# automl/mdp-playground

Measured on AMD Instinct MI355X. Metric: env-steps/sec, higher is better.
Workload: dtype u8; 1 GPU; cfg2: BASELINE configs[1]: discrete 8x8, delay 4, sequence_length 3; 65536 envs/GPU, random actions, same-step autoreset; 1 bench step = 1 fused launch of 512 env steps; envs_per_gpu=65536, fuse=512, env_steps_per_bench_step=33554432, rng=numpy, collective=all_gather_into_tensor(nccl, 1 rank) after every launch

## Files before the change

mdp_playground_amd/csrc/mdpp_discrete_lean.hip:

```cpp
#include <stdlib.h>

#include <stdio.h>

#include <type_traits>

#ifndef MDPP_LEAN_TU_NEXT
#define MDPP_LEAN_TU_NEXT 0
#endif
#ifndef MDPP_LEAN_TU_NOISE
#define MDPP_LEAN_TU_NOISE 0
#endif

#include "mdpp_internal.hpp"
#include "mdpp_rng.hpp"

namespace mdpp {

#ifndef MDPP_LEAN_CHUNK
#define MDPP_LEAN_CHUNK 8
#endif
#ifndef MDPP_LEAN_DEPTH
#define MDPP_LEAN_DEPTH 32
#endif
#ifndef MDPP_LEAN_AHEAD
#define MDPP_LEAN_AHEAD 4
#endif
#if defined(MDPP_LEAN_PRIO_E) || defined(MDPP_LEAN_PRIO_O) || defined(MDPP_LEAN_PRIO_H)
#define MDPP_LEAN_PRIO_FORCED 1
#else
#define MDPP_LEAN_PRIO_FORCED 0
#endif
#ifndef MDPP_LEAN_PRIO_E
#define MDPP_LEAN_PRIO_E 3
#endif
#ifndef MDPP_LEAN_PRIO_O
#define MDPP_LEAN_PRIO_O 2
#endif
#ifndef MDPP_LEAN_PRIO_H
#define MDPP_LEAN_PRIO_H 0
#endif
#ifndef MDPP_LEAN_PRIO_O2
#define MDPP_LEAN_PRIO_O2 -1
#endif
#ifndef MDPP_LEAN_ST_AUX
#define MDPP_LEAN_ST_AUX MDPP_ST_NT
#endif
#ifndef MDPP_LEAN_ST_AUX_BYTES
#define MDPP_LEAN_ST_AUX_BYTES MDPP_LEAN_ST_AUX
#endif
#ifndef MDPP_LEAN_LD_AUX
#define MDPP_LEAN_LD_AUX 0
#endif
#ifndef MDPP_LEAN_HMIN
#define MDPP_LEAN_HMIN 16
#endif
#ifndef MDPP_LEAN_HSLEEP
#define MDPP_LEAN_HSLEEP 8
#endif
namespace lean {
constexpr int kChunk = MDPP_LEAN_CHUNK;
constexpr int kDepth = MDPP_LEAN_DEPTH;
constexpr int kAhead = MDPP_LEAN_AHEAD;
constexpr int kPRsrc = 0x00020000;
constexpr uint32_t kSpinLimit = 1u << 22;
constexpr uint32_t kStatusInternal = 0x80000000u;
constexpr uint32_t kQueueCap = 6;
constexpr int kHChunks = 8;
constexpr int kHChunksNp = 4;
constexpr int kXR = 16;
constexpr int kXB = 4;
constexpr int kDepthNp = 16;
constexpr int kRoles = 4;
constexpr uint32_t kSelPad = 0x0c0c0c00u;
typedef unsigned int u32x2 __attribute__((ext_vector_type(2)));
typedef unsigned int u32x4 __attribute__((ext_vector_type(4)));

__device__ __forceinline__ uint32_t wg_load_acq(const uint32_t *p) {
    return __hip_atomic_load(p, __ATOMIC_ACQUIRE, __HIP_MEMORY_SCOPE_WORKGROUP);
}
__device__ __forceinline__ void wg_store_rel(uint32_t *p, uint32_t v) {
    __hip_atomic_store(p, v, __ATOMIC_RELEASE, __HIP_MEMORY_SCOPE_WORKGROUP);
}
__device__ __forceinline__ void chunk_words(uint64_t seed, uint64_t genv, uint64_t b0, uint32_t r4, uint32_t stream,
                                            uint32_t (&wd)[MDPP_LEAN_CHUNK]) {
    uint32_t o0[4], o1[4], o2[4] = {0u, 0u, 0u, 0u};
    philox_start_block(seed, genv, b0, stream, o0);
    philox_start_block(seed, genv, b0 + 1, stream, o1);
    if (r4 != 0u) philox_start_block(seed, genv, b0 + 2, stream, o2);
    const uint32_t all[12] = {o0[0], o0[1], o0[2], o0[3], o1[0], o1[1], o1[2], o1[3], o2[0], o2[1], o2[2], o2[3]};
#pragma unroll
// ... 4 lines not shown
                                              float (&z)[MDPP_LEAN_CHUNK]) {
    float all[12] = {0.0f, 0.0f, 0.0f, 0.0f, 0.0f, 0.0f, 0.0f, 0.0f, 0.0f, 0.0f, 0.0f, 0.0f};
    uint32_t o[4];
    philox_start_block(seed, genv, b0, stream, o);
    philox_box_muller2(o, all[0], all[1], all[2], all[3]);
    philox_start_block(seed, genv, b0 + 1, stream, o);
    philox_box_muller2(o, all[4], all[5], all[6], all[7]);
    if (r4 != 0u) {
        philox_start_block(seed, genv, b0 + 2, stream, o);
        philox_box_muller2(o, all[8], all[9], all[10], all[11]);
    }
#pragma unroll
    for (int u = 0; u < MDPP_LEAN_CHUNK; u++)
        z[u] = r4 == 0u ? all[u] : r4 == 1u ? all[u + 1] : r4 == 2u ? all[u + 2] : all[u + 3];
}
}
using namespace lean;

template <bool OBS64, bool DELAY, bool HASMAX, bool EVN, bool PHILOX, bool IRR, bool NEXT, int NZ = 0>
__global__ __launch_bounds__(kRoles * kBlock) void k_discrete_rollout_lean(DiscreteArgs a, int K,
                                                                      const int32_t *__restrict__ actions,
                                                                      void *__restrict__ obs,
                                                                      float *__restrict__ reward,
                                                                      uint8_t *__restrict__ term,
                                                                      uint8_t *__restrict__ trunc,
                                                                      void *__restrict__ final_obs) {
    const uint64_t ptick0 = tick_now(a);
    constexpr bool PN = (NZ & 1) != 0, RN = (NZ & 2) != 0;
    constexpr bool NPN = PN && !PHILOX, NRN = RN && !PHILOX;
    constexpr bool Z0 = (NZ & 4) != 0;
    static_assert(!Z0 || NRN, "sigma-0 draws: numpy streams with the reward_noise key");
    constexpr bool NRX = NRN && !Z0;
    constexpr int KD = NRN ? kDepthNp : kDepth;
    __shared__ __align__(16) uint32_t lds_rec[3][KD][kBlock];
    __shared__ __align__(16) uint32_t lds_V[2048];
    __shared__ __align__(16) uint2 lds_col[16];
    __shared__ __align__(16) uint32_t lds_R[128];
    __shared__ __align__(16) uint64_t lds_T[8];
    __shared__ __align__(16) float lds_rsel[EVN ? 4 * 64 : 4];
    __shared__ __align__(16) uint64_t lds_ring[kBlock];
    __shared__ uint32_t lds_head[kBlock];
    __shared__ uint32_t lds_prod[kBlock / 64];
    __shared__ __align__(8) uint32_t lds_cons[kBlock / 64][2];
    __shared__ uint32_t lds_done;
    constexpr bool ROWS2 = !IRR && NZ == 0;
    constexpr bool ROWS1 = ROWS2 && !PHILOX;
    constexpr int kRB = 4;
    __shared__ __align__(16) float lds_rw[ROWS1 ? kRB : 1][kChunk][ROWS1 ? kBlock : 4];
    __shared__ __align__(16) uint32_t lds_rprod[kBlock / 64], lds_rcons[kBlock / 64];
    typedef typename std::conditional<IRR, uint64_t, uint32_t>::type S0Word;
    __shared__ __align__(16) S0Word lds_s0[PHILOX ? kHChunks : 1][kBlock];
    __shared__ __align__(16) uint2 lds_col1[IRR ? 16 : 1];
    __shared__ __align__(16) uint64_t lds_T1[IRR ? 8 : 1];
    __shared__ uint32_t lds_hprod[kBlock / 64];
    __shared__ uint32_t lds_pprod[kBlock / 64];
    constexpr bool kNpNoise = !PHILOX && NZ != 0;
    constexpr bool kPhNoise = PHILOX && NZ != 0;
    constexpr int kPrioE = MDPP_LEAN_PRIO_FORCED ? MDPP_LEAN_PRIO_E : kNpNoise ? 2 : !PHILOX ? MDPP_LEAN_PRIO_E : 1;
    constexpr int kPrioO = MDPP_LEAN_PRIO_FORCED ? MDPP_LEAN_PRIO_O : kNpNoise ? 1 : !PHILOX ? MDPP_LEAN_PRIO_O : kPhNoise ? 2 : (PN ? 2 : 3);
    constexpr int kPrioH = MDPP_LEAN_PRIO_FORCED ? MDPP_LEAN_PRIO_H : kNpNoise ? 3 : !PHILOX ? MDPP_LEAN_PRIO_H : kPhNoise ? 2 : (PN ? 3 : 2);
    static_assert(NZ == 0 || (!IRR && !NEXT), "noise on the lean kernel: one sub-space, same-step autoreset");
    __shared__ __align__(16) uint32_t lds_pn[(PN && PHILOX) ? kHChunks : 1][kBlock];
    __shared__ __align__(16) uint32_t lds_pn2[NPN ? kHChunksNp : 1][2][kBlock];
    __shared__ __align__(16) double lds_x[NRX ? kXR : 1][kBlock];
    __shared__ uint16_t lds_meta[NRN ? kXR : 1][kBlock];
    __shared__ __align__(16) double lds_rx[NRX ? KD : 1][kBlock];
    __shared__ uint32_t lds_hhead[NRN ? kBlock : 1], lds_epos[NRN ? kBlock : 1];
    __shared__ uint8_t lds_sstab[(NRN || NPN) ? 2048 : 1];
    __shared__ uint8_t lds_pntab[NPN ? 4096 : 1];
    __shared__ ulonglong2 lds_kw[NRN ? 256 : 1];
    __shared__ double lds_fi[NRN ? 256 : 1];
    constexpr int kEN = IRR ? 2 : 1;
    constexpr bool nextmode = NEXT;
    const bool ar = a.autoreset != 0;
    const int tid = threadIdx.x;
    const int role = tid / kBlock;
    const int l = tid & (kBlock - 1);
    const int w = l >> 6;
    const uint32_t S = (uint32_t)a.S, L = (uint32_t)a.L;
    if (tid < 16) {
        uint64_t cs = 0;
        if (tid < a.A)
            for (uint32_t s = 0; s < S; s++) {
                const uint32_t nx = a.P[s * a.A + tid] & 7u;
                cs |= (uint64_t)(nx | 8u | ((uint32_t)((a.term_mask >> nx) & 1ULL) << 7)) << (8 * s);
            }
        lds_col[tid] = make_uint2((uint32_t)cs, (uint32_t)(cs >> 32));
        if (tid < 8) lds_T[tid] = a.init_thr[tid];
        if (IRR) {
            uint64_t c1 = 0;
            if (tid < a.A1)
                for (int s1 = 0; s1 < a.S1; s1++) c1 |= (uint64_t)(a.P1[s1 * a.A1 + tid] & 7u) << (8 * s1);
            lds_col1[tid] = make_uint2((uint32_t)c1, (uint32_t)(c1 >> 32));
            if (tid < 8) lds_T1[tid] = tid < a.S1 ? (uint64_t)ceil(a.init_cdf1[tid] * 9007199254740992.0) : ~0ULL;
        }
        if (!EVN && tid < 4) lds_rsel[tid] = a.rsel[tid];
    }
    if (EVN)
        for (int k = tid; k < 4 * a.every_n; k += kRoles * kBlock) lds_rsel[k] = a.rsel[k < 4 ? k : (k & 1)];
    for (uint32_t k = tid; k < 128; k += kRoles * kBlock) {
        uint32_t wd = 0;
        for (int b = 0; b < 4; b++) {
            uint32_t byte = 4 * k + b;
            if (byte < a.rbits_stride) wd |= (uint32_t)a.rbits[byte] << (8 * b);
        }
        lds_R[k] = wd;
    }
    if (tid < kBlock) { lds_ring[tid] = 0; lds_head[tid] = 0; if (NRN) { lds_hhead[tid] = 0; lds_epos[tid] = 0; } }
    if (NRN || NPN) {
        for (uint32_t k = tid; k < 2048u; k += kRoles * kBlock) {
            const uint64_t lo = (uint64_t)k << 53, hi = lo + ((1ULL << 53) - 1ULL);
            uint32_t c0 = 0, c1 = 0;
            for (int j = 0; j < 8; j++) {
                const uint64_t t = a.init_thr[j] > (1ULL << 53) - 1ULL ? ~0ULL : a.init_thr[j] << 11;
                c0 += (t <= lo) ? 1u : 0u; c1 += (t <= hi) ? 1u : 0u;
            }
            lds_sstab[k] = (uint8_t)(c0 == c1 ? c0 : 0xFFu);
        }
    }
    if (NPN) {
        for (uint32_t k = tid; k < 4096u; k += kRoles * kBlock) {
            const uint64_t lo = (uint64_t)k << 52, hi = lo + ((1ULL << 52) - 1ULL);
            uint32_t a0 = 0, a1 = 0, b0 = 0, b1 = 0;
            for (int j = 0; j < 7; j++) { a0 += (a.pn_TL[j] <= lo) ? 1u : 0u; a1 += (a.pn_TL[j] <= hi) ? 1u : 0u; }
            for (int j = 0; j < 8; j++) { b0 += (a.pn_TU[j] <= lo) ? 1u : 0u; b1 += (a.pn_TU[j] <= hi) ? 1u : 0u; }
            lds_pntab[k] = (uint8_t)((a0 == a1 && b0 == b1) ? (a0 | (b0 << 4)) : 0xFFu);
        }
    }
    if (NRN)
        for (int k = tid; k < 256; k += kRoles * kBlock) { lds_kw[k] = make_ulonglong2(d_zig_ki[k], (unsigned long long)(__double_as_longlong(d_zig_wi[k]) + (52LL << 52)));    lds_fi[k] = d_zig_fi[k]; }
    if (tid < kBlock / 64) { lds_prod[tid] = 0; lds_cons[tid][0] = 0; lds_cons[tid][1] = 0; lds_hprod[tid] = 0; lds_pprod[tid] = 0; lds_rprod[tid] = 0; lds_rcons[tid] = 0; }
    if (tid == 0) lds_done = 0;
    __syncthreads();
    {
        uint32_t dmask = 0;
        for (uint32_t j = 1; j <= L; j++) dmask |= 1u << (4 * j - 2);
        for (uint32_t d = tid; d < 2048; d += kRoles * kBlock) {
            uint32_t wd = 0;
            if ((d & dmask) == dmask) {
                for (uint32_t b = 8; b < 32; b++) {
                    if (!(b & 8u)) continue;
                    const uint32_t idx = d * 32u + b;
// ... 5 lines not shown
            lds_V[d] = wd;
        }
    }
    uint32_t steps_at_launch = 0;
    {
        const uint32_t eb0 = ((gridDim.x & 7u) == 0u) ? (blockIdx.x & 7u) * (gridDim.x >> 3) + (blockIdx.x >> 3) : blockIdx.x;
        const uint32_t i0 = eb0 * kBlock + l;
        if (EVN && role == 1 && i0 < (uint32_t)a.N) steps_at_launch = ((const uint32_t *)&a.state[i0])[2] & 0x7FFFFFFFu;
    }
    __syncthreads();

    const uint32_t eblk = ((gridDim.x & 7u) == 0u) ? (blockIdx.x & 7u) * (gridDim.x >> 3) + (blockIdx.x >> 3) : blockIdx.x;
    const uint32_t i = eblk * kBlock + l;
    const uint32_t N = (uint32_t)a.N;
    const bool rows = ROWS2 && (N % (uint32_t)kBlock) == 0u;
    const uint32_t blk0 = eblk * kBlock, ln = (uint32_t)l & 63u;
    const uint32_t ws = (uint32_t)__builtin_amdgcn_readfirstlane(w);
    auto min4 = [&](const uint32_t *p) -> uint32_t {
        const uint64_t x = __hip_atomic_load((const uint64_t *)p, __ATOMIC_ACQUIRE, __HIP_MEMORY_SCOPE_WORKGROUP);
        const uint64_t y = __hip_atomic_load((const uint64_t *)p + 1, __ATOMIC_ACQUIRE, __HIP_MEMORY_SCOPE_WORKGROUP);
        return min(min((uint32_t)x, (uint32_t)(x >> 32)), min((uint32_t)y, (uint32_t)(y >> 32)));
    };
    if (i >= N) {
        if (role == 0 && (l & 63) == 0) __hip_atomic_fetch_add(&lds_done, 1u, __ATOMIC_RELEASE, __HIP_MEMORY_SCOPE_WORKGROUP);
        return;
    }
    const uint32_t A = (uint32_t)a.A;
    constexpr int kMinLanes = MDPP_LEAN_HMIN;
    uint32_t status = 0;

    if (role == 3) {
        if (!ar && !PN && !NRN) return;
        __builtin_amdgcn_s_setprio(kPrioH);
        if constexpr (PHILOX) {
            const uint64_t genv = (uint64_t)(a.env_id_offset + (int64_t)i);
            const int nch = (K + kChunk - 1) / kChunk;
            static_assert(kChunk == 8, "two start-state blocks per chunk");
            uint32_t thr[8], thr1[8];
#pragma unroll
            for (int j = 0; j < 8; j++) {
                const uint64_t t53 = lds_T[j];
                thr[j] = __builtin_amdgcn_readfirstlane(t53 > (1ULL << 53) ? 0x80000000u : (uint32_t)((t53 + 0x3FFFFFULL) >> 22));
                const uint64_t u53 = IRR ? lds_T1[j] : ~0ULL;
                thr1[j] = __builtin_amdgcn_readfirstlane(u53 > (1ULL << 53) ? 0x80000000u : (uint32_t)((u53 + 0x3FFFFFULL) >> 22));
            }
            const uint32_t r4 = (uint32_t)ptick0 & 3u;
            for (int c = 0; c < nch; c++) {
                if (c >= kHChunks) {
                    const uint32_t must = (uint32_t)min((c - kHChunks + 1) * kChunk, K);
                    uint32_t spins = 0;
                    while (wg_load_acq(&lds_prod[w]) < must) {
                        __builtin_amdgcn_s_sleep(2);
                        if (++spins > kSpinLimit) { status |= kStatusInternal; break; }
                    }
                }
                const uint64_t b0 = (ptick0 + (uint64_t)(c * kChunk)) >> 2;
                auto words = [&](uint32_t stream, uint32_t (&wd)[kChunk]) { chunk_words(a.philox_seed, genv, b0, r4, stream, wd); };
                uint32_t wd[kChunk], wd1[kChunk];
                words(kPhiloxStartStream, wd);
                if (IRR) words(kPhiloxStartIrrStream, wd1);
                S0Word pk = 0;
#pragma unroll
                for (int u = 0; u < kChunk; u++) {
                    const uint32_t m = wd[u] >> 1;
                    uint32_t s0 = 0;
#pragma unroll
                    for (int j = 0; j < 7; j++) s0 += (thr[j] <= m) ? 1u : 0u;
                    if (IRR) {
                        const uint32_t m1 = wd1[u] >> 1;
                        uint32_t s1 = 0;
#pragma unroll
                        for (int j = 0; j < 7; j++) s1 += (thr1[j] <= m1) ? 1u : 0u;
                        s0 |= (s1 | 8u) << 4;
                    }
                    pk |= (S0Word)(s0 | 8u) << (kEN * 4 * u);
                }
                lds_s0[c % kHChunks][l] = pk;
                if ((l & 63) == 0) wg_store_rel(&lds_hprod[w], (uint32_t)(c + 1));
            }
            if (status) atomicOr(&a.status[i], status);
            return;
        }
        if constexpr (NPN || NRN) {
            Pcg64 g;
            g.load(a.env_s, a.env_inc, i);
            Pcg64LimbsLo ge;
            ge.from(g);
            uint32_t hq = 0;
            uint64_t look = 0;
            if (NRN) look = ge.next64();
            uint32_t vals = 0, tail = 0, spins = 0;
            auto start_of = [&](uint64_t r) __attribute__((always_inline)) -> uint32_t {
                uint32_t s0 = lds_sstab[(uint32_t)(r >> 53)];
                if (__builtin_expect(__builtin_amdgcn_ballot_w64(s0 == 0xFFu) != 0, 0)) {
                    if (s0 == 0xFFu) {
                        const uint64_t m = r >> 11;
                        s0 = 0;
#pragma unroll
                        for (int j = 0; j < 8; j++) s0 += (a.init_thr[j] <= m) ? 1u : 0u;
                    }
                }
                return s0;
            };
            for (;;) {
                if (wg_load_acq(&lds_done) == kBlock / 64) break;
                bool did = false;
                if constexpr (NRN) {
                    const uint32_t epos = __hip_atomic_load(&lds_epos[l], __ATOMIC_RELAXED, __HIP_MEMORY_SCOPE_WORKGROUP);
                    const bool go = hq + (uint32_t)kXB <= epos + (uint32_t)kXR;
                    if (__builtin_amdgcn_ballot_w64(go) != 0) {
                        uint32_t rej = 0;
                        uint64_t wdv[kXB + 1];
                        if (go) {
                            wdv[0] = look;
#pragma unroll
                            for (int u = 0; u < kXB; u++) {
                                const uint64_t wd = wdv[u];
                                wdv[u + 1] = ge.next64();
                                const uint64_t rabs = (wd >> 9) & 0x000fffffffffffffULL;
                                if constexpr (Z0) {
                                    const uint64_t ki = lds_kw[(uint32_t)wd & 0xffu].x;
                                    const bool ok = rabs < ki;
                                    rej |= ok ? 0u : (1u << u);
                                    lds_meta[(hq + (uint32_t)u) & (uint32_t)(kXR - 1)][l] = (uint16_t)(start_of(wd) | (ok ? 0u : (2u << 3)));
                                    continue;
                                }
                                const ulonglong2 kw = lds_kw[(uint32_t)wd & 0xffu];
                                const double W = __longlong_as_double((long long)kw.y);
                                const double x = __builtin_fma(__longlong_as_double((long long)(rabs | 0x3FF0000000000000ULL)), W, -W);
                                const uint64_t xb = (uint64_t)__double_as_longlong(x);
                                const double xs = __longlong_as_double((long long)(((uint64_t)(((uint32_t)(xb >> 32) & 0x7FFFFFFFu) |
                                                                                   (((uint32_t)wd << 23) & 0x80000000u)) << 32) | (uint32_t)xb));
                                const bool ok = rabs < kw.x;
                                rej |= ok ? 0u : (1u << u);
                                const uint32_t slot = (hq + (uint32_t)u) & (uint32_t)(kXR - 1);
                                lds_x[slot][l] = xs;
// ... 77 lines not shown
                            tail += 1u;
                        }
                        __hip_atomic_store(&lds_ring[l], (uint64_t)vals | ((uint64_t)tail << 32), __ATOMIC_RELEASE,
                                           __HIP_MEMORY_SCOPE_WORKGROUP);
                        did = true;
                    }
                }
                if (__builtin_amdgcn_ballot_w64(did) == 0) {
                    __builtin_amdgcn_s_sleep(2);
                    if (++spins > kSpinLimit * 4u) { status |= kStatusInternal; break; }
                } else {
                    spins = 0;
                }
            }
            auto undraw = [&](Pcg64 &gg, uint32_t q) {
                for (; q > 0; q--) {
                    uint64_t lo = gg.s_lo - gg.inc_lo;
                    uint64_t hi = gg.s_hi - gg.inc_hi - (gg.s_lo < gg.inc_lo ? 1ULL : 0ULL);
                    gg.s_lo = lo * a.minv_lo;
                    gg.s_hi = __umul64hi(lo, a.minv_lo) + lo * a.minv_hi + hi * a.minv_lo;
                }
            };
            ge.to(g);
            if (NRN) undraw(g, hq + 1u - __hip_atomic_load(&lds_epos[l], __ATOMIC_ACQUIRE, __HIP_MEMORY_SCOPE_WORKGROUP));
            else undraw(g, tail - wg_load_acq(&lds_head[l]));
            g.store(a.env_s, i);
            if (status) atomicOr(&a.status[i], status);
            return;
        }
        Pcg64 g;
        g.load(a.env_s, a.env_inc, i);
        auto draw = [&](Pcg64 &gg) -> uint32_t {
            const uint64_t r0 = gg.next64();
            const uint64_t m = r0 >> 11;
            uint32_t s0 = 0;
#pragma unroll
            for (int j = 0; j < 8; j++) s0 += (lds_T[j] <= m) ? 1u : 0u;
            if (IRR) {
                const uint64_t m1 = gg.next64() >> 11;
                uint32_t s1 = 0;
#pragma unroll
                for (int j = 0; j < 8; j++) s1 += (lds_T1[j] <= m1) ? 1u : 0u;
                s0 |= (s1 | 8u) << 4;
            }
            return s0;
        };
        uint32_t vals = 0, tail = 0;
        for (;;) {
            if (wg_load_acq(&lds_done) == kBlock / 64) break;
            const uint32_t head = wg_load_acq(&lds_head[l]);
            const uint32_t cnt = tail - head;
            const bool want = cnt + (uint32_t)kEN <= 8u;
            const uint64_t bw = __builtin_amdgcn_ballot_w64(want);
            const bool urgent = __builtin_amdgcn_ballot_w64(want && cnt <= 2) != 0;
            if (__builtin_popcountll(bw) >= kMinLanes || urgent) {
                Pcg64 n = g;
                const uint32_t s0 = draw(n) | 8u;
                if (want) {
                    const uint32_t sh = (tail & 7u) * 4u;
                    g = n;
                    vals = (vals & ~((IRR ? 0xFFu : 0xFu) << sh)) | (s0 << sh);
                    tail += (uint32_t)kEN;
                }
                __hip_atomic_store(&lds_ring[l], (uint64_t)vals | ((uint64_t)tail << 32), __ATOMIC_RELEASE,
                                   __HIP_MEMORY_SCOPE_WORKGROUP);
            } else {
                __builtin_amdgcn_s_sleep(MDPP_LEAN_HSLEEP);
            }
        }
        const uint32_t head = wg_load_acq(&lds_head[l]);
        for (uint32_t q = tail - head; q > 0; q--) {
            uint64_t lo = g.s_lo - g.inc_lo;
            uint64_t hi = g.s_hi - g.inc_hi - (g.s_lo < g.inc_lo ? 1ULL : 0ULL);
            g.s_lo = lo * a.minv_lo;
            g.s_hi = __umul64hi(lo, a.minv_lo) + lo * a.minv_hi + hi * a.minv_lo;
        }
        g.store(a.env_s, i);
        return;
    }

    const uint32_t total = (uint32_t)K * N;
    const int nchunks = (K + kChunk - 1) / kChunk;

    if (role == 1) {
        __builtin_amdgcn_s_setprio(kPrioO);
        auto r_rew = __builtin_amdgcn_make_buffer_rsrc((void *)reward, 0, total * 4u, kPRsrc);
        const uint32_t v4 = i * 4u;
        const uint32_t dsh = (uint32_t)(a.delay > 0 ? a.delay - 1 : 0);
        uint32_t ring = ((const uint32_t *)&a.state[i])[3];
        const uint8_t *rselb = (const uint8_t *)lds_rsel;

        const uint32_t ph_full = 16u * (uint32_t)a.every_n;
        uint32_t ph = EVN ? ph_full - 16u * (steps_at_launch % (uint32_t)a.every_n) : 0u;
        const uint64_t genv = (uint64_t)(a.env_id_offset + (int64_t)i);
        const uint32_t r4 = (uint32_t)ptick0 & 3u;
        float zc[kChunk] = {0.0f, 0.0f, 0.0f, 0.0f, 0.0f, 0.0f, 0.0f, 0.0f};
        const bool plain = a.scale == 1.0 && a.shift == 0.0;
        auto emit = [&](uint32_t ra, uint32_t rb, uint32_t rc, uint32_t so, double z, float *stage) {
            uint32_t bit = lds_V[(ra >> 5) & 2047u] >> (ra & 31u);
            uint32_t out;
            if (DELAY) {
                out = (ring >> dsh) & 1u;
                ring = (ring << 1) | (bit & 1u);
                ring = (ra != rb) ? 0u : ring;
            } else {
                out = bit & 1u;
            }
            const uint32_t tb = (rc >> 7) & 1u;
            uint32_t rd = 0;
            if (EVN) {
                ph -= 16u;
                rd = ph;
                ph = (ra != rb || ph == 0u) ? ph_full : ph;
            }
            float rout;
            if constexpr (RN && !Z0) {
                double r = (out != 0u && (!EVN || rd == 0u)) ? 1.0 : 0.0;
                r += 0.0 + a.r_noise * z;
                if (!plain) {
                    r *= a.scale;
                    r += a.shift;
                }
                if (tb) r += a.term_add;
                rout = (float)r;
            } else {
                rout = EVN ? *(const float *)(rselb + (rd | (out << 3) | (tb << 2)))
                           : *(const float *)(rselb + (((out << 1) | tb) << 2));
            }
            if (nextmode) rout = (ra != rb) ? 0.0f : rout;
            if (stage) { *stage = rout; return; }
            __builtin_amdgcn_raw_buffer_store_b32(__float_as_uint(rout), r_rew, v4, so * 4u, MDPP_LEAN_ST_AUX);
        };
        for (int c = 0; c < nchunks; c++) {
            const int kbase = c * kChunk;
            const uint32_t upto = (uint32_t)min(kbase + kChunk, K);
            if constexpr (RN && PHILOX)
                chunk_normals(a.philox_seed, genv, (ptick0 + (uint64_t)kbase) >> 2, r4, kPhiloxRNoiseStream, zc);
            uint32_t spins = 0;
            while (wg_load_acq(&lds_prod[w]) < upto) {
                __builtin_amdgcn_s_sleep(1);
                if (++spins > kSpinLimit) { status |= kStatusInternal; break; }
            }
            const bool rowc = ROWS1 && rows && kbase + kChunk <= K;
            if (kbase + kChunk <= K) {
                uint32_t ra[kChunk], rb[kChunk], rc[kChunk];
#pragma unroll
                for (int u = 0; u < kChunk; u++) {
                    ra[u] = lds_rec[0][(kbase + u) % KD][l];
                    rb[u] = lds_rec[1][(kbase + u) % KD][l];
                    rc[u] = lds_rec[2][(kbase + u) % KD][l];
                }
                double zd[kChunk];
#pragma unroll
                for (int u = 0; u < kChunk; u++) zd[u] = NRX ? lds_rx[NRX ? (kbase + u) % KD : 0][l] : (double)zc[u];
                if (rowc && c >= kRB) {
                    uint32_t sp2 = 0;
                    while (min4(lds_rcons) < (uint32_t)(c - kRB + 1)) {
                        __builtin_amdgcn_s_sleep(1);
                        if (++sp2 > kSpinLimit) { status |= kStatusInternal; break; }
                    }
                }
#pragma unroll
                for (int u = 0; u < kChunk; u++)
                    emit(ra[u], rb[u], rc[u], (uint32_t)(kbase + u) * N, zd[u], rowc ? &lds_rw[ROWS1 ? (c % kRB) : 0][u][ROWS1 ? l : 0] : nullptr);
            } else {
#pragma unroll
                for (int u = 0; u < kChunk; u++)
                    if (kbase + u < K)
                        emit(lds_rec[0][(kbase + u) % KD][l], lds_rec[1][(kbase + u) % KD][l],
                             lds_rec[2][(kbase + u) % KD][l], (uint32_t)(kbase + u) * N,
                             NRX ? lds_rx[NRX ? (kbase + u) % KD : 0][l] : (double)zc[u], nullptr);
            }
            if ((l & 63) == 0) wg_store_rel(&lds_cons[w][0], upto);
            if constexpr (ROWS1) {
                if (rowc && (l & 63) == 0) wg_store_rel(&lds_rprod[w], (uint32_t)(c + 1));
            }
        }
        ((uint32_t *)&a.state[i])[3] = ring;
        if (status) atomicOr(&a.status[i], status);
        return;
    }

    if (role == 2) {
        __builtin_amdgcn_s_setprio(MDPP_LEAN_PRIO_O2 >= 0 ? MDPP_LEAN_PRIO_O2 : (NPN && !MDPP_LEAN_PRIO_FORCED) ? (NRN ? 2 : 3)
                                   : (PN && PHILOX && !MDPP_LEAN_PRIO_FORCED) ? (RN ? 2 : 3) : kPrioO);
        auto r_obs = __builtin_amdgcn_make_buffer_rsrc(obs, 0, total * (OBS64 ? 8u : 4u) * (uint32_t)kEN, kPRsrc);
        auto r_term = __builtin_amdgcn_make_buffer_rsrc((void *)term, 0, total, kPRsrc);
        auto r_rew2 = __builtin_amdgcn_make_buffer_rsrc((void *)reward, 0, total * 4u, kPRsrc);
        auto r_trunc = __builtin_amdgcn_make_buffer_rsrc((void *)trunc, 0, total, kPRsrc);
        const uint32_t v1 = i, v4 = i * 4u, v8 = i * 8u, v16 = i * 16u;
        auto emit = [&](uint32_t rb, uint32_t rc, uint32_t so) {
            const uint32_t o = rb & 7u;
            if (IRR) {
                const uint32_t o1 = (rc >> 8) & 7u;
                if (OBS64) __builtin_amdgcn_raw_buffer_store_b128(u32x4{o, 0u, o1, 0u}, r_obs, v16 + so * 16u, 0, MDPP_LEAN_ST_AUX);
                else __builtin_amdgcn_raw_buffer_store_b64(u32x2{o, o1}, r_obs, v8, so * 8u, MDPP_LEAN_ST_AUX);
            } else if (OBS64) __builtin_amdgcn_raw_buffer_store_b64(u32x2{o, 0u}, r_obs, v8, so * 8u, MDPP_LEAN_ST_AUX);
            else __builtin_amdgcn_raw_buffer_store_b32(o, r_obs, v4, so * 4u, MDPP_LEAN_ST_AUX);
            __builtin_amdgcn_raw_buffer_store_b8((uint8_t)((rc >> 7) & 1u), r_term, v1, so, MDPP_LEAN_ST_AUX_BYTES);
            __builtin_amdgcn_raw_buffer_store_b8(HASMAX ? (uint8_t)(rc >> 16) : (uint8_t)0, r_trunc, v1, so, MDPP_LEAN_ST_AUX_BYTES);
        };
        Pcg64 sp;
// ... 188 lines not shown
        }
        if constexpr (NRN) return;
        if (!PHILOX && !ar) return;
        if constexpr (PHILOX) {
            uint32_t spins = 0;
            while (wg_load_acq(&lds_hprod[w]) < (uint32_t)(c + 1)) {
                __builtin_amdgcn_s_sleep(1);
                if (++spins > kSpinLimit) { status |= kStatusInternal; break; }
            }
            s0c = lds_s0[c % kHChunks][l];
            if constexpr (PN) {
                spins = 0;
                while (wg_load_acq(&lds_pprod[w]) < (uint32_t)(c + 1)) {
                    __builtin_amdgcn_s_sleep(1);
                    if (++spins > kSpinLimit) { status |= kStatusInternal; break; }
                }
                pnc = lds_pn[c % kHChunks][l];
            }
            return;
        }
        const uint64_t rt = __hip_atomic_load(&lds_ring[l], __ATOMIC_ACQUIRE, __HIP_MEMORY_SCOPE_WORKGROUP);
        const uint32_t vals = (uint32_t)rt, tail = (uint32_t)(rt >> 32);
        const uint32_t qc = (uint32_t)__builtin_popcount(qv & 0x88888888u);
        const uint32_t avail = tail - head_local, room = kQueueCap - qc;
        const uint32_t take = avail < room ? avail : room;
        const uint32_t rot = __builtin_amdgcn_alignbit(vals, vals, (head_local & 7u) * 4u);
        const uint32_t m = (1u << (4u * take)) - 1u;
        qv |= (rot & m) << (4u * qc);
        head_local += take;
        __hip_atomic_store(&lds_head[l], head_local, __ATOMIC_RELAXED, __HIP_MEMORY_SCOPE_WORKGROUP);
    };
    typedef typename std::conditional<IRR, uint2, int>::type Act;
    typedef typename std::conditional<IRR, uint4, uint2>::type Col;
    auto column = [&](Act act, uint32_t &badm, int u) -> Col {
        int action;
        if constexpr (IRR) action = (int)act.x; else action = act;
        uint32_t ua = (uint32_t)action;
        if (__builtin_expect(__builtin_amdgcn_ballot_w64(ua >= A) != 0, 0)) {
            ua = (uint32_t)(action + ((action >> 31) & (int)A));
            const bool bad = ua >= A;
            if (nextmode) badm |= bad ? (1u << u) : 0u; else status |= bad ? (uint32_t)MDPP_STATUS_BAD_ACTION : 0u;
            ua = bad ? 0u : ua;
        }
        if constexpr (IRR) {
            const int action1 = (int)act.y;
            uint32_t ub = (uint32_t)action1;
            if (__builtin_expect(__builtin_amdgcn_ballot_w64(ub >= A1) != 0, 0)) {
                ub = (uint32_t)(action1 + ((action1 >> 31) & (int)A1));
                const bool bad = ub >= A1;
                if (nextmode) badm |= bad ? (1u << u) : 0u; else status |= bad ? (uint32_t)MDPP_STATUS_BAD_ACTION : 0u;
                ub = bad ? 0u : ub;
            }
            const uint2 ca = lds_col[ua], cb = lds_col1[ub];
            return make_uint4(ca.x, ca.y, cb.x, cb.y);
        } else {
            return lds_col[ua];
        }
    };
    auto stepE = [&](const Col &col, int k, uint32_t badbit) {
        uint32_t entry = __builtin_amdgcn_perm(col.y, col.x, sel);
        if constexpr (PN && PHILOX) {
            const uint32_t nib = (pnc >> (4 * (k % kChunk))) & 0xFu, j = nib & 7u, nx = entry & 7u;
            const uint32_t ns = nib > 7u ? j + (j >= nx ? 1u : 0u) : nx;
            entry = __builtin_amdgcn_perm(enc_hi, enc_lo, ns | kSelPad);
        }
        if constexpr (NPN) {
            const uint32_t by = (((k % kChunk) < 4 ? pnc : pnc_hi) >> (8 * (k & 3))) & 0xFFu, nx = entry & 7u;
            const uint32_t ns = min(by & 15u, nx) + (uint32_t)max((int)(by >> 4) - (int)nx, 0);
            entry = __builtin_amdgcn_perm(enc_hi, enc_lo, ns | kSelPad);
        }
        const uint32_t k2n = (k2 << 4) | entry;
        bool need = entry > 0x7Fu;
        uint32_t rc = entry;
        if (HASMAX) {
            cnt += 1;
            need = need || cnt >= 0x10000u;
            rc = __builtin_amdgcn_perm(cnt, entry, 0x0c060c00u);
        }
        need = need && ar;
        uint32_t rec_a = k2n;
        if (nextmode) {
            const bool ended = need && !pend;
            need = pend;
            rc = pend ? 0u : rc;
            rec_a = pend ? 0u : k2n;
            status |= (badbit != 0u && !pend) ? (uint32_t)MDPP_STATUS_BAD_ACTION : 0u;
            pend = ended;
        }
        uint32_t s0v = PHILOX ? (uint32_t)(s0c >> (kEN * 4 * (k % kChunk))) & (IRR ? 0xFFu : 0xFu) : qv & (IRR ? 0xFFu : 0xFu);
        if constexpr (NRN) {
            uint32_t kind = (m0 >> 3) & 3u;
            if (__builtin_expect(__builtin_amdgcn_ballot_w64(kind >= 2u) != 0, 0)) {
                uint32_t guard = 0;
                while (__builtin_amdgcn_ballot_w64(kind == 2u) != 0) {
                    const bool red = kind == 2u;
                    ep += red ? 2u : 0u;
                    uint32_t o0 = m0, o1 = m1, o2 = m2;
                    double ox = xv;
                    fetch();
                    if (!red) { m0 = o0; m1 = o1; m2 = o2; xv = ox; }
                    kind = (m0 >> 3) & 3u;
                    if (++guard > 64u) { status |= kStatusInternal; break; }
                }
            }
            uint32_t cntw = kind == 0u ? 1u : 2u, ssm = kind == 0u ? m1 : m2;
            if (kind == 3u) { cntw = m0 >> 8; ssm = m0 >> 5; }
            if constexpr (NRX) lds_rx[k % KD][l] = xv;
            s0v = (ssm & 7u) | 8u;
            ep += cntw + (need ? 1u : 0u);
            __hip_atomic_store(&lds_epos[l], ep, __ATOMIC_RELAXED, __HIP_MEMORY_SCOPE_WORKGROUP);
            fetch();
        }
        if (!PHILOX && !NRN && __builtin_expect(__builtin_amdgcn_ballot_w64(need && s0v == 0u) != 0, 0)) {
            uint32_t spins = 0;
            while (__builtin_amdgcn_ballot_w64(need && (qv & 0xFu) == 0u) != 0) {
                pull(-1);
                __builtin_amdgcn_s_sleep(1);
                if (++spins > kSpinLimit) { status |= kStatusInternal; qv |= 8u; break; }
            }
            s0v = qv & (IRR ? 0xFFu : 0xFu);
        }
        if constexpr (IRR) {
            const uint32_t n1 = __builtin_amdgcn_perm(col.w, col.z, c1 | kSelPad);
            c1 = need ? ((s0v >> 4) & 7u) : n1;
            rc |= c1 << 8;
            s0v &= 0xFu;
        }
        k2 = need ? s0v : k2n;
        if (!PHILOX && !NRN) qv = need ? (qv >> (4 * kEN)) : qv;
        if (HASMAX) cnt = need ? c0 : cnt;
        else last_reset = need ? (uint32_t)(k + 1) : last_reset;
        sel = (k2 & 7u) | kSelPad;
        lds_rec[0][k % KD][l] = rec_a;
        lds_rec[1][k % KD][l] = k2;
        lds_rec[2][k % KD][l] = rc;
    };

    auto load_act = [&](int k) -> Act {
        const uint32_t kk = (uint32_t)min(k, K - 1);
        if constexpr (IRR) {
            const u32x2 v = __builtin_amdgcn_raw_buffer_load_b64(r_act, v4, kk * N * 8u, MDPP_LEAN_LD_AUX);
            return make_uint2(v.x, v.y);
        } else {
            return __builtin_amdgcn_raw_buffer_load_b32(r_act, v4, kk * N * 4u, MDPP_LEAN_LD_AUX);
        }
    };
    constexpr int kAh = IRR ? 2 : kAhead;
    static_assert(kAh % 2 == 0, "the column double buffer alternates with the chunk index");
    Act actq[kAh][kChunk];
    Col colq[2][kChunk];
#pragma unroll
    for (int u = 0; u < kChunk; u++) colq[0][u] = column(load_act(u), badq[0], u);
#pragma unroll
    for (int q = 0; q < kAh; q++)
#pragma unroll
        for (int u = 0; u < kChunk; u++) actq[q][u] = load_act((q + 1) * kChunk + u);

    const int nfull = K / kChunk;
    auto wait_room = [&](int kend) {
        if (kend > KD) {
            const uint32_t must = (uint32_t)(kend - KD);
            uint32_t spins = 0;
            for (;;) {
                const uint64_t cc = __hip_atomic_load((const uint64_t *)&lds_cons[w][0], __ATOMIC_ACQUIRE,
                                                      __HIP_MEMORY_SCOPE_WORKGROUP);
                uint32_t have = min((uint32_t)cc, (uint32_t)(cc >> 32));
                if (rows) {
#pragma unroll
                    for (int j = 0; j < kBlock / 64; j++) have = min(have, wg_load_acq(&lds_cons[j][1]));
                }
                if (have >= must) break;
                __builtin_amdgcn_s_sleep(1);
                if (++spins > kSpinLimit) { status |= kStatusInternal; break; }
            }
        }
    };
    auto chunkE = [&](int c, int j, bool refill) {
        const int kbase = c * kChunk;
        badq[(j + 1) & 1] = 0u;
#pragma unroll
        for (int u = 0; u < kChunk; u++) colq[(j + 1) & 1][u] = column(actq[j][u], badq[(j + 1) & 1], u);
        if (refill) {
#pragma unroll
            for (int u = 0; u < kChunk; u++) actq[j][u] = load_act(kbase + (kAh + 1) * kChunk + u);
        }
        wait_room(kbase + kChunk);
        pull(c);
#pragma unroll
        for (int u = 0; u < kChunk; u++) stepE(colq[j & 1][u], kbase + u, (badq[j & 1] >> u) & 1u);
        if (NRN) __hip_atomic_store(&lds_epos[l], ep, __ATOMIC_RELAXED, __HIP_MEMORY_SCOPE_WORKGROUP);
        if ((l & 63) == 0) wg_store_rel(&lds_prod[w], (uint32_t)(kbase + kChunk));
    };
    const int ngrp = nfull / kAh;
    for (int g = 0; g < ngrp; g++) {
#pragma unroll
        for (int j = 0; j < kAh; j++) chunkE(g * kAh + j, j, true);
    }
#pragma unroll
    for (int j = 0; j < kAh - 1; j++)
        if (ngrp * kAh + j < nfull) chunkE(ngrp * kAh + j, j, false);
    if (K % kChunk) {
        const int kbase = nfull * kChunk;
        Act ta[kChunk];
#pragma unroll
        for (int u = 0; u < kChunk; u++) ta[u] = load_act(kbase + u);
        wait_room(kbase + kChunk);
        pull(nfull);
#pragma unroll
        for (int u = 0; u < kChunk; u++)
            if (kbase + u < K) {
                uint32_t bm = 0;
                const Col cc = column(ta[u], bm, 0);
                stepE(cc, kbase + u, bm);
            }
        if ((l & 63) == 0) wg_store_rel(&lds_prod[w], (uint32_t)K);
    }

    uint32_t hist = 0;
    for (int j = 3; j >= 0; j--) {
        const uint32_t nb = (k2 >> (4 * j)) & 0xFu;
        hist = (hist << 8) | ((nb & 8u) ? (nb & 7u) : 0xFFu);
    }
    const uint32_t qc = (uint32_t)__builtin_popcount(qv & 0x00888888u);
    const bool own_q = !PHILOX && !IRR && !nextmode && NZ == 0;
    if (NRN) __hip_atomic_store(&lds_epos[l], ep, __ATOMIC_RELEASE, __HIP_MEMORY_SCOPE_WORKGROUP);
    if (!own_q && !PHILOX && !NRN) {
        __hip_atomic_store(&lds_head[l], head_local - qc, __ATOMIC_RELEASE, __HIP_MEMORY_SCOPE_WORKGROUP);
    }
    if (IRR) a.irr_state[i] = c1;
    uint32_t steps;
    if (HASMAX) steps = cnt - c0;
    else steps = last_reset ? (uint32_t)K - last_reset : steps0 + (uint32_t)K;
    uint32_t *st = (uint32_t *)&a.state[i];
    st[0] = hist; st[2] = steps | (pend ? 0x80000000u : 0u);
    if (own_q) st[1] = (qv & 0x00777777u) | (qc << 24);
    if ((l & 63) == 0) __hip_atomic_fetch_add(&lds_done, 1u, __ATOMIC_RELEASE, __HIP_MEMORY_SCOPE_WORKGROUP);
    if (status) atomicOr(&a.status[i], status);
}

static bool lean_launch(const DiscreteArgs &a, const DiscreteIO &io, const int nz) {
    constexpr bool kNext = MDPP_LEAN_TU_NEXT;
    const int K = io.K;
    const bool ph = a.philox != 0, irr = a.irr != 0;
    if (io.final_obs) return false;
    const bool shape = a.autoreset == MDPP_AUTORESET_NEXT_STEP ? a.lean_next_ok != 0
                       : (nz && !ph) ? a.shape_ok_noise_np != 0
// ... 69 lines not shown
```

Baseline: 261.8 billion env-steps/s.

## Hoist per-step checks to chunk level, table-lookup start states, restructure LDS

The environment-step role now checks action range once per chunk and runs the step loop speculatively without the per-step queue-empty check. If any lane found its start-state queue empty, it restores the saved state and replays the chunk with full checks. The numpy reset draw uses a precomputed 2048-entry start-state table in LDS instead of an 8-way threshold compare. LDS is packed into one struct with big buffers placed last, and the reward emit path gets compile-time staging variants. The speculative replay adds code size and register pressure in exchange for fewer ballots in the common path.

```diff
diff --git a/mdp_playground_amd/csrc/mdpp_discrete_lean.hip b/mdp_playground_amd/csrc/mdpp_discrete_lean.hip
--- a/mdp_playground_amd/csrc/mdpp_discrete_lean.hip
+++ b/mdp_playground_amd/csrc/mdpp_discrete_lean.hip
@@ -56,6 +56,15 @@
 #endif
 #ifndef MDPP_LEAN_HSLEEP
 #define MDPP_LEAN_HSLEEP 8
+#endif
+#ifndef MDPP_LEAN_E_CHUNK_TEST
+#define MDPP_LEAN_E_CHUNK_TEST 1
+#endif
+#ifndef MDPP_LEAN_H_TABLE
+#define MDPP_LEAN_H_TABLE 1
+#endif
+#ifndef MDPP_LEAN_O1_STRAIGHT
+#define MDPP_LEAN_O1_STRAIGHT 1
 #endif
 namespace lean {
 constexpr int kChunk = MDPP_LEAN_CHUNK;
@@ -126,45 +135,62 @@
     static_assert(!Z0 || NRN, "sigma-0 draws: numpy streams with the reward_noise key");
     constexpr bool NRX = NRN && !Z0;
     constexpr int KD = NRN ? kDepthNp : kDepth;
-    __shared__ __align__(16) uint32_t lds_rec[3][KD][kBlock];
-    __shared__ __align__(16) uint32_t lds_V[2048];
-    __shared__ __align__(16) uint2 lds_col[16];
-    __shared__ __align__(16) uint32_t lds_R[128];
-    __shared__ __align__(16) uint64_t lds_T[8];
-    __shared__ __align__(16) float lds_rsel[EVN ? 4 * 64 : 4];
-    __shared__ __align__(16) uint64_t lds_ring[kBlock];
-    __shared__ uint32_t lds_head[kBlock];
-    __shared__ uint32_t lds_prod[kBlock / 64];
-    __shared__ __align__(8) uint32_t lds_cons[kBlock / 64][2];
-    __shared__ uint32_t lds_done;
     constexpr bool ROWS2 = !IRR && NZ == 0;
     constexpr bool ROWS1 = ROWS2 && !PHILOX;
     constexpr int kRB = 4;
-    __shared__ __align__(16) float lds_rw[ROWS1 ? kRB : 1][kChunk][ROWS1 ? kBlock : 4];
-    __shared__ __align__(16) uint32_t lds_rprod[kBlock / 64], lds_rcons[kBlock / 64];
     typedef typename std::conditional<IRR, uint64_t, uint32_t>::type S0Word;
-    __shared__ __align__(16) S0Word lds_s0[PHILOX ? kHChunks : 1][kBlock];
-    __shared__ __align__(16) uint2 lds_col1[IRR ? 16 : 1];
-    __shared__ __align__(16) uint64_t lds_T1[IRR ? 8 : 1];
-    __shared__ uint32_t lds_hprod[kBlock / 64];
-    __shared__ uint32_t lds_pprod[kBlock / 64];
     constexpr bool kNpNoise = !PHILOX && NZ != 0;
     constexpr bool kPhNoise = PHILOX && NZ != 0;
     constexpr int kPrioE = MDPP_LEAN_PRIO_FORCED ? MDPP_LEAN_PRIO_E : kNpNoise ? 2 : !PHILOX ? MDPP_LEAN_PRIO_E : 1;
     constexpr int kPrioO = MDPP_LEAN_PRIO_FORCED ? MDPP_LEAN_PRIO_O : kNpNoise ? 1 : !PHILOX ? MDPP_LEAN_PRIO_O : kPhNoise ? 2 : (PN ? 2 : 3);
     constexpr int kPrioH = MDPP_LEAN_PRIO_FORCED ? MDPP_LEAN_PRIO_H : kNpNoise ? 3 : !PHILOX ? MDPP_LEAN_PRIO_H : kPhNoise ? 2 : (PN ? 3 : 2);
     static_assert(NZ == 0 || (!IRR && !NEXT), "noise on the lean kernel: one sub-space, same-step autoreset");
-    __shared__ __align__(16) uint32_t lds_pn[(PN && PHILOX) ? kHChunks : 1][kBlock];
-    __shared__ __align__(16) uint32_t lds_pn2[NPN ? kHChunksNp : 1][2][kBlock];
-    __shared__ __align__(16) double lds_x[NRX ? kXR : 1][kBlock];
-    __shared__ uint16_t lds_meta[NRN ? kXR : 1][kBlock];
-    __shared__ __align__(16) double lds_rx[NRX ? KD : 1][kBlock];
-    __shared__ uint32_t lds_hhead[NRN ? kBlock : 1], lds_epos[NRN ? kBlock : 1];
-    __shared__ uint8_t lds_sstab[(NRN || NPN) ? 2048 : 1];
-    __shared__ uint8_t lds_pntab[NPN ? 4096 : 1];
-    __shared__ ulonglong2 lds_kw[NRN ? 256 : 1];
-    __shared__ double lds_fi[NRN ? 256 : 1];
     constexpr int kEN = IRR ? 2 : 1;
+    constexpr bool HTAB = NRN || NPN || (MDPP_LEAN_H_TABLE && !PHILOX && NZ == 0);
+    struct Lds {
+#if !MDPP_LEAN_O1_STRAIGHT
+        __align__(16) uint32_t rec[3][KD][kBlock];
+        __align__(16) float rw[ROWS1 ? kRB : 1][kChunk][ROWS1 ? kBlock : 4];
+#endif
+        __align__(16) uint32_t V[2048];
+        __align__(16) float rsel[EVN ? 4 * 64 : 4];
+        __align__(16) uint2 col[16];
+        __align__(16) uint2 col1[IRR ? 16 : 1];
+        __align__(16) uint32_t R[128];
+        __align__(16) uint64_t T[8];
+        __align__(16) uint64_t T1[IRR ? 8 : 1];
+        uint8_t sstab[HTAB ? 2048 : 1];
+        uint8_t pntab[NPN ? 4096 : 1];
+        __align__(16) ulonglong2 kw[NRN ? 256 : 1];
+        double fi[NRN ? 256 : 1];
+        __align__(16) uint32_t prod[kBlock / 64];
+        __align__(8) uint32_t cons[kBlock / 64][2];
+        __align__(16) uint32_t rprod[kBlock / 64], rcons[kBlock / 64];
+        uint32_t hprod[kBlock / 64];
+        uint32_t pprod[kBlock / 64];
+        uint32_t done;
+        __align__(16) uint64_t ring[kBlock];
+        uint32_t head[kBlock];
+        uint32_t hhead[NRN ? kBlock : 1], epos[NRN ? kBlock : 1];
+        __align__(16) S0Word s0[PHILOX ? kHChunks : 1][PHILOX ? kBlock : 1];
+        __align__(16) uint32_t pn[(PN && PHILOX) ? kHChunks : 1][(PN && PHILOX) ? kBlock : 1];
+        __align__(16) uint32_t pn2[NPN ? kHChunksNp : 1][2][NPN ? kBlock : 1];
+        uint16_t meta[NRN ? kXR : 1][NRN ? kBlock : 1];
+        __align__(16) double x[NRX ? kXR : 1][NRX ? kBlock : 1];
+        __align__(16) double rx[NRX ? KD : 1][NRX ? kBlock : 1];
+#if MDPP_LEAN_O1_STRAIGHT
+        __align__(16) float rw[ROWS1 ? kRB : 1][kChunk][ROWS1 ? kBlock : 4];
+        __align__(16) uint32_t rec[3][KD][kBlock];
+#endif
+    };
+    static_assert(sizeof(Lds) <= 160 * 1024, "the workgroup's LDS");
+    __shared__ Lds sm;
+    auto &lds_rec = sm.rec; auto &lds_rw = sm.rw; auto &lds_V = sm.V; auto &lds_rsel = sm.rsel; auto &lds_col = sm.col; auto &lds_col1 = sm.col1;
+    auto &lds_R = sm.R; auto &lds_T = sm.T; auto &lds_T1 = sm.T1; auto &lds_sstab = sm.sstab; auto &lds_pntab = sm.pntab; auto &lds_kw = sm.kw;
+    auto &lds_fi = sm.fi; auto &lds_prod = sm.prod; auto &lds_cons = sm.cons; auto &lds_rprod = sm.rprod; auto &lds_rcons = sm.rcons;
+    auto &lds_hprod = sm.hprod; auto &lds_pprod = sm.pprod; auto &lds_done = sm.done; auto &lds_ring = sm.ring; auto &lds_head = sm.head;
+    auto &lds_hhead = sm.hhead; auto &lds_epos = sm.epos; auto &lds_s0 = sm.s0; auto &lds_pn = sm.pn; auto &lds_pn2 = sm.pn2;
+    auto &lds_meta = sm.meta; auto &lds_x = sm.x; auto &lds_rx = sm.rx;
     constexpr bool nextmode = NEXT;
     const bool ar = a.autoreset != 0;
     const int tid = threadIdx.x;
@@ -201,7 +227,7 @@
         lds_R[k] = wd;
     }
     if (tid < kBlock) { lds_ring[tid] = 0; lds_head[tid] = 0; if (NRN) { lds_hhead[tid] = 0; lds_epos[tid] = 0; } }
-    if (NRN || NPN) {
+    if (HTAB) {
         for (uint32_t k = tid; k < 2048u; k += kRoles * kBlock) {
             const uint64_t lo = (uint64_t)k << 53, hi = lo + ((1ULL << 53) - 1ULL);
             uint32_t c0 = 0, c1 = 0;
@@ -273,6 +299,18 @@
     if (role == 3) {
         if (!ar && !PN && !NRN) return;
         __builtin_amdgcn_s_setprio(kPrioH);
+        auto start_of = [&](uint64_t r) __attribute__((always_inline)) -> uint32_t {
+            uint32_t s0 = lds_sstab[(uint32_t)(r >> 53)];
+            if (__builtin_expect(__builtin_amdgcn_ballot_w64(s0 == 0xFFu) != 0, 0)) {
+                if (s0 == 0xFFu) {
+                    const uint64_t m = r >> 11;
+                    s0 = 0;
+#pragma unroll
+                    for (int j = 0; j < 8; j++) s0 += (lds_T[j] <= m) ? 1u : 0u;
+                }
+            }
+            return s0;
+        };
         if constexpr (PHILOX) {
             const uint64_t genv = (uint64_t)(a.env_id_offset + (int64_t)i);
             const int nch = (K + kChunk - 1) / kChunk;
@@ -331,18 +369,6 @@
             uint64_t look = 0;
             if (NRN) look = ge.next64();
             uint32_t vals = 0, tail = 0, spins = 0;
-            auto start_of = [&](uint64_t r) __attribute__((always_inline)) -> uint32_t {
-                uint32_t s0 = lds_sstab[(uint32_t)(r >> 53)];
-                if (__builtin_expect(__builtin_amdgcn_ballot_w64(s0 == 0xFFu) != 0, 0)) {
-                    if (s0 == 0xFFu) {
-                        const uint64_t m = r >> 11;
-                        s0 = 0;
-#pragma unroll
-                        for (int j = 0; j < 8; j++) s0 += (a.init_thr[j] <= m) ? 1u : 0u;
-                    }
-                }
-                return s0;
-            };
             for (;;) {
                 if (wg_load_acq(&lds_done) == kBlock / 64) break;
                 bool did = false;
@@ -486,10 +512,14 @@
         g.load(a.env_s, a.env_inc, i);
         auto draw = [&](Pcg64 &gg) -> uint32_t {
             const uint64_t r0 = gg.next64();
-            const uint64_t m = r0 >> 11;
             uint32_t s0 = 0;
-#pragma unroll
-            for (int j = 0; j < 8; j++) s0 += (lds_T[j] <= m) ? 1u : 0u;
+            if constexpr (HTAB) {
+                s0 = start_of(r0);
+            } else {
+                const uint64_t m = r0 >> 11;
+#pragma unroll
+                for (int j = 0; j < 8; j++) s0 += (lds_T[j] <= m) ? 1u : 0u;
+            }
             if (IRR) {
                 const uint64_t m1 = gg.next64() >> 11;
                 uint32_t s1 = 0;
@@ -550,7 +580,7 @@
         const uint32_t r4 = (uint32_t)ptick0 & 3u;
         float zc[kChunk] = {0.0f, 0.0f, 0.0f, 0.0f, 0.0f, 0.0f, 0.0f, 0.0f};
         const bool plain = a.scale == 1.0 && a.shift == 0.0;
-        auto emit = [&](uint32_t ra, uint32_t rb, uint32_t rc, uint32_t so, double z, float *stage) {
+        auto emit = [&](auto STAGE, uint32_t ra, uint32_t rb, uint32_t rc, uint32_t so, double z, float *stage) __attribute__((always_inline)) {
             uint32_t bit = lds_V[(ra >> 5) & 2047u] >> (ra & 31u);
             uint32_t out;
             if (DELAY) {
@@ -582,8 +612,9 @@
                            : *(const float *)(rselb + (((out << 1) | tb) << 2));
             }
             if (nextmode) rout = (ra != rb) ? 0.0f : rout;
-            if (stage) { *stage = rout; return; }
-            __builtin_amdgcn_raw_buffer_store_b32(__float_as_uint(rout), r_rew, v4, so * 4u, MDPP_LEAN_ST_AUX);
+            if constexpr (STAGE() < 0) { if (stage) { *stage = rout; return; } }
+            if constexpr (STAGE() > 0) *stage = rout;
+            else __builtin_amdgcn_raw_buffer_store_b32(__float_as_uint(rout), r_rew, v4, so * 4u, MDPP_LEAN_ST_AUX);
         };
         for (int c = 0; c < nchunks; c++) {
             const int kbase = c * kChunk;
@@ -614,14 +645,24 @@
                         if (++sp2 > kSpinLimit) { status |= kStatusInternal; break; }
                     }
                 }
-#pragma unroll
-                for (int u = 0; u < kChunk; u++)
-                    emit(ra[u], rb[u], rc[u], (uint32_t)(kbase + u) * N, zd[u], rowc ? &lds_rw[ROWS1 ? (c % kRB) : 0][u][ROWS1 ? l : 0] : nullptr);
+                if (!MDPP_LEAN_O1_STRAIGHT) {
+#pragma unroll
+                    for (int u = 0; u < kChunk; u++)
+                        emit(std::integral_constant<int, -1>{}, ra[u], rb[u], rc[u], (uint32_t)(kbase + u) * N, zd[u], rowc ? &lds_rw[ROWS1 ? (c % kRB) : 0][u][ROWS1 ? l : 0] : nullptr);
+                } else if (rowc) {
+#pragma unroll
+                    for (int u = 0; u < kChunk; u++)
+                        emit(std::integral_constant<int, 1>{}, ra[u], rb[u], rc[u], 0u, zd[u], &lds_rw[ROWS1 ? (c % kRB) : 0][u][ROWS1 ? l : 0]);
+                } else {
+#pragma unroll
+                    for (int u = 0; u < kChunk; u++)
+                        emit(std::integral_constant<int, 0>{}, ra[u], rb[u], rc[u], (uint32_t)(kbase + u) * N, zd[u], nullptr);
+                }
             } else {
 #pragma unroll
                 for (int u = 0; u < kChunk; u++)
                     if (kbase + u < K)
-                        emit(lds_rec[0][(kbase + u) % KD][l], lds_rec[1][(kbase + u) % KD][l],
+                        emit(std::integral_constant<int, 0>{}, lds_rec[0][(kbase + u) % KD][l], lds_rec[1][(kbase + u) % KD][l],
                              lds_rec[2][(kbase + u) % KD][l], (uint32_t)(kbase + u) * N,
                              NRX ? lds_rx[NRX ? (kbase + u) % KD : 0][l] : (double)zc[u], nullptr);
             }
@@ -876,11 +917,11 @@
     };
     typedef typename std::conditional<IRR, uint2, int>::type Act;
     typedef typename std::conditional<IRR, uint4, uint2>::type Col;
-    auto column = [&](Act act, uint32_t &badm, int u) -> Col {
+    auto column = [&](auto RANGE, Act act, uint32_t &badm, int u) __attribute__((always_inline)) -> Col {
         int action;
         if constexpr (IRR) action = (int)act.x; else action = act;
         uint32_t ua = (uint32_t)action;
-        if (__builtin_expect(__builtin_amdgcn_ballot_w64(ua >= A) != 0, 0)) {
+        if (RANGE() && __builtin_expect(__builtin_amdgcn_ballot_w64(ua >= A) != 0, 0)) {
             ua = (uint32_t)(action + ((action >> 31) & (int)A));
             const bool bad = ua >= A;
             if (nextmode) badm |= bad ? (1u << u) : 0u; else status |= bad ? (uint32_t)MDPP_STATUS_BAD_ACTION : 0u;
@@ -901,7 +942,9 @@
             return lds_col[ua];
         }
     };
-    auto stepE = [&](const Col &col, int k, uint32_t badbit) {
+    constexpr bool ECHUNK = MDPP_LEAN_E_CHUNK_TEST && !PHILOX && NZ == 0 && !IRR && !NEXT;
+    uint32_t fed = 8u, lr8 = 0u;
+    auto stepE = [&](auto CHK, const Col &col, int k, int u, uint32_t badbit) __attribute__((always_inline)) {
         uint32_t entry = __builtin_amdgcn_perm(col.y, col.x, sel);
         if constexpr (PN && PHILOX) {
             const uint32_t nib = (pnc >> (4 * (k % kChunk))) & 0xFu, j = nib & 7u, nx = entry & 7u;
@@ -955,7 +998,8 @@
             __hip_atomic_store(&lds_epos[l], ep, __ATOMIC_RELAXED, __HIP_MEMORY_SCOPE_WORKGROUP);
             fetch();
         }
-        if (!PHILOX && !NRN && __builtin_expect(__builtin_amdgcn_ballot_w64(need && s0v == 0u) != 0, 0)) {
+        if constexpr (!CHK()) {
+        } else if (!PHILOX && !NRN && __builtin_expect(__builtin_amdgcn_ballot_w64(need && s0v == 0u) != 0, 0)) {
             uint32_t spins = 0;
             while (__builtin_amdgcn_ballot_w64(need && (qv & 0xFu) == 0u) != 0) {
                 pull(-1);
@@ -971,8 +1015,10 @@
             s0v &= 0xFu;
         }
         k2 = need ? s0v : k2n;
+        if constexpr (!CHK()) fed &= k2;
         if (!PHILOX && !NRN) qv = need ? (qv >> (4 * kEN)) : qv;
         if (HASMAX) cnt = need ? c0 : cnt;
+        else if constexpr (!CHK()) lr8 = need ? (uint32_t)(u + 1) : lr8;
         else last_reset = need ? (uint32_t)(k + 1) : last_reset;
         sel = (k2 & 7u) | kSelPad;
         lds_rec[0][k % KD][l] = rec_a;
@@ -994,7 +1040,7 @@
     Act actq[kAh][kChunk];
     Col colq[2][kChunk];
 #pragma unroll
-    for (int u = 0; u < kChunk; u++) colq[0][u] = column(load_act(u), badq[0], u);
+    for (int u = 0; u < kChunk; u++) colq[0][u] = column(std::true_type{}, load_act(u), badq[0], u);
 #pragma unroll
     for (int q = 0; q < kAh; q++)
 #pragma unroll
@@ -1006,7 +1052,7 @@
             const uint32_t must = (uint32_t)(kend - KD);
             uint32_t spins = 0;
             for (;;) {
-                const uint64_t cc = __hip_atomic_load((const uint64_t *)&lds_cons[w][0], __ATOMIC_ACQUIRE,
+                const uint64_t cc = __hip_atomic_load((const uint64_t *)&sm.cons[w][0], __ATOMIC_ACQUIRE,
                                                       __HIP_MEMORY_SCOPE_WORKGROUP);
                 uint32_t have = min((uint32_t)cc, (uint32_t)(cc >> 32));
                 if (rows) {
@@ -1019,19 +1065,47 @@
             }
         }
     };
-    auto chunkE = [&](int c, int j, bool refill) {
+    auto chunkE = [&](int c, int j, bool refill) __attribute__((always_inline)) {
         const int kbase = c * kChunk;
         badq[(j + 1) & 1] = 0u;
-#pragma unroll
-        for (int u = 0; u < kChunk; u++) colq[(j + 1) & 1][u] = column(actq[j][u], badq[(j + 1) & 1], u);
+        if constexpr (ECHUNK) {
+            uint32_t amax = 0;
+#pragma unroll
+            for (int u = 0; u < kChunk; u++) amax = max(amax, (uint32_t)actq[j][u]);
+            if (__builtin_expect(__builtin_amdgcn_ballot_w64(amax >= A) != 0, 0)) {
+#pragma unroll
+                for (int u = 0; u < kChunk; u++) colq[(j + 1) & 1][u] = column(std::true_type{}, actq[j][u], badq[(j + 1) & 1], u);
+            } else {
+#pragma unroll
+                for (int u = 0; u < kChunk; u++) colq[(j + 1) & 1][u] = column(std::false_type{}, actq[j][u], badq[(j + 1) & 1], u);
+            }
+        } else {
+#pragma unroll
+            for (int u = 0; u < kChunk; u++) colq[(j + 1) & 1][u] = column(std::true_type{}, actq[j][u], badq[(j + 1) & 1], u);
+        }
         if (refill) {
 #pragma unroll
             for (int u = 0; u < kChunk; u++) actq[j][u] = load_act(kbase + (kAh + 1) * kChunk + u);
         }
         wait_room(kbase + kChunk);
         pull(c);
-#pragma unroll
-        for (int u = 0; u < kChunk; u++) stepE(colq[j & 1][u], kbase + u, (badq[j & 1] >> u) & 1u);
+        if constexpr (ECHUNK) {
+            const uint32_t k2_0 = k2, qv_0 = qv, cnt_0 = cnt;
+            fed = 8u; lr8 = 0u;
+#pragma unroll
+            for (int u = 0; u < kChunk; u++) stepE(std::false_type{}, colq[j & 1][u], kbase + u, u, 0u);
+            if (__builtin_expect(__builtin_amdgcn_ballot_w64((fed & 8u) == 0u) != 0, 0)) {
+                k2 = k2_0; qv = qv_0; cnt = cnt_0;
+                sel = (k2 & 7u) | kSelPad;
+#pragma unroll
+                for (int u = 0; u < kChunk; u++) stepE(std::true_type{}, colq[j & 1][u], kbase + u, u, 0u);
+            } else if (!HASMAX) {
+                last_reset = lr8 != 0u ? (uint32_t)kbase + lr8 : last_reset;
+            }
+        } else {
+#pragma unroll
+            for (int u = 0; u < kChunk; u++) stepE(std::true_type{}, colq[j & 1][u], kbase + u, u, (badq[j & 1] >> u) & 1u);
+        }
         if (NRN) __hip_atomic_store(&lds_epos[l], ep, __ATOMIC_RELAXED, __HIP_MEMORY_SCOPE_WORKGROUP);
         if ((l & 63) == 0) wg_store_rel(&lds_prod[w], (uint32_t)(kbase + kChunk));
     };
@@ -1054,8 +1128,8 @@
         for (int u = 0; u < kChunk; u++)
             if (kbase + u < K) {
                 uint32_t bm = 0;
-                const Col cc = column(ta[u], bm, 0);
-                stepE(cc, kbase + u, bm);
+                const Col cc = column(std::true_type{}, ta[u], bm, 0);
+                stepE(std::true_type{}, cc, kbase + u, u, bm);
             }
         if ((l & 63) == 0) wg_store_rel(&lds_prod[w], (uint32_t)K);
     }
```

Result: no change. 262.8 billion env-steps/s (median of 6 runs) (+0.4%).
